# elte-collective-intelligence/student-mechanism-design

Measured on NVIDIA B200. Metric: batched_env_steps_per_sec, higher is better.
Workload: dtype int32/f64

## Files before the change

### include/sy_env.h

```cpp
#ifndef SY_ENV_H
#define SY_ENV_H

#include <stdint.h>

#ifdef __cplusplus
extern "C" {
#endif

#define SY_ABI_VERSION 4
#define SY_NUM_REWARD_WEIGHTS 11
#define SY_MAX_AGENTS 16
#define SY_NUM_STATS 16
#define SY_MAX_COPY_SEGMENTS 8
#define SY_DEFAULT_ACTION (-1)

enum {
  SY_OK = 0,
  SY_ERR_INVALID_ARGUMENT = 1,
  SY_ERR_CUDA = 2,
  SY_ERR_STATE = 3
};

enum { SY_REWARD_FP64 = 0, SY_REWARD_FP32 = 1 };
enum { SY_STATUS_TERMINATED = 1, SY_STATUS_TRUNCATED = 2, SY_STATUS_FROZEN = 4 };
// ... 67 lines not shown
  int32_t* mrx_revealed;
  uint8_t* node_features_u8;
} SyObs;

typedef struct SyOut {
  uint64_t struct_bytes;
  float* reward;
  double* reward64;
  uint8_t* terminated;
  uint8_t* truncated;
  uint8_t* done;
  int8_t* winner;
  int64_t* stats;
  uint8_t* status;
} SyOut;

int sy_abi_version(void);
const char* sy_last_error(void);
int64_t sy_launch_count(void);

int sy_create(const SyConfig* config, SyEnv** out_env);
void sy_destroy(SyEnv* env);
enum { SY_OPT_WRITER_PATH = 0, SY_OPT_STEP_KERNEL = 1, SY_OPT_NF_FILL = 2, SY_OPT_LAGGED_KERNEL = 3, SY_OPT_TAIL_SPLIT = 4,
       SY_OPT_ROLLOUT_KERNEL = 5, SY_OPT_PDL = 6 };
enum { SY_WRITER_BULK = 0, SY_WRITER_LSU = 1 };
enum { SY_STEP_FUSED = 0, SY_STEP_TWO_KERNELS = 1, SY_STEP_AUTO = 2 };
enum { SY_LAGGED_OFF = 0, SY_LAGGED_ON = 1, SY_LAGGED_AUTO = 2 };
int sy_set_option(SyEnv* env, int32_t option, int32_t value);
int sy_set_seed(SyEnv* env, uint64_t seed);

int sy_set_reward_tables(SyEnv* env, const double* exp_neg, int32_t n_exp, const double* coverage,
                         int32_t n_cov, sy_stream_t stream);

int sy_load_graphs(SyEnv* env, int32_t num_graphs, const int32_t* row_ptr, const int32_t* col,
                   const int32_t* w, int32_t nnz_stride, sy_stream_t stream);
int sy_generate_graphs(SyEnv* env, int32_t num_graphs, int32_t num_edges, int32_t max_edges_per_node, int32_t max_weight,
                       uint64_t seed, uint32_t generation, uint32_t graph_offset, int32_t* attempts_host,
                       sy_stream_t stream);
int sy_read_graph_edges(SyEnv* env, int32_t* edge_links, int32_t* weights, int32_t* counts, int32_t max_edges,
                        sy_stream_t stream);
int sy_read_graph_tables(SyEnv* env, int32_t g, uint8_t* weights, uint16_t* apsp, sy_stream_t stream);

int sy_reset(SyEnv* env, const uint8_t* reset_mask, const int32_t* init_pos, const int32_t* init_graph_id,
             int32_t restart, const SyState* state, const SyObs* obs, sy_stream_t stream);

int sy_step(SyEnv* env, const int64_t* actions, const SyState* state, const SyObs* obs, const SyOut* out,
            sy_stream_t stream);

int sy_step_deferred(SyEnv* env, const int64_t* actions, const SyState* state, const SyObs* obs, const SyOut* out,
                     sy_stream_t stream);
int sy_flush_observations(SyEnv* env, const SyState* state, const SyObs* obs, sy_stream_t stream);
int sy_observations_pending(SyEnv* env);

typedef struct SyHostOut {
  uint64_t struct_bytes;
  float* reward;
  uint8_t* terminated;
  uint8_t* truncated;
  uint8_t* done;
  int8_t* winner;
  uint8_t* status;
} SyHostOut;

int sy_step_host(SyEnv* env, const int64_t* actions_host, int64_t* actions_dev, const SyState* state,
                 const SyObs* obs, const SyOut* out, const SyHostOut* host_out, sy_stream_t stream);

int sy_step_i32(SyEnv* env, const int32_t* actions, const SyState* state, const SyObs* obs, const SyOut* out,
                sy_stream_t stream);
int sy_step_i16(SyEnv* env, const int16_t* actions, const SyState* state, const SyObs* obs, const SyOut* out,
                sy_stream_t stream);
int sy_step_host_i16(SyEnv* env, const int16_t* actions_host, int16_t* actions_dev, const SyState* state,
                     const SyObs* obs, const SyOut* out, const SyHostOut* host_out, sy_stream_t stream);
int sy_sample_actions_i16(SyEnv* env, const SyState* state, uint32_t step_counter, int16_t* actions,
                          sy_stream_t stream);
int sy_set_host_overlap(SyEnv* env, int32_t on);
// ... 46 lines not shown
```

### student_mechanism_design_b200/_cabi.py

```python
from __future__ import annotations

import ctypes as C
import os

_HERE = os.path.dirname(os.path.abspath(__file__))
LIB_PATH = os.environ.get("SY_LIB_PATH") or os.path.join(_HERE, "libsy_env.so")

SY_ABI_VERSION = 4
SY_NUM_REWARD_WEIGHTS = 11
SY_MAX_AGENTS = 16
SY_NUM_STATS = 16
SY_MAX_GROUPS = 1024
SY_REWARD_FP64, SY_REWARD_FP32 = 0, 1
STAT_NAMES = [
    "env_steps", "episodes", "mrx_wins", "police_wins", "truncations", "out_of_money",
    "sum_episode_length", "sum_budget_spent", "sum_sq_episode_length", "sum_length_police_wins",
    "sum_length_mrx_wins", "sum_episode_budget_spent", "police_moves",
    "reveals", "sum_belief_ce_q24", "sum_sq_belief_ce_q24",
]
BELIEF_CE_SCALE = float(1 << 24)


class SyConfig(C.Structure):
    _fields_ = [
# ... 45 lines not shown
    "sy_launch_count": (C.c_int64, []),
    "sy_create": (C.c_int, [C.POINTER(SyConfig), C.POINTER(C.c_void_p)]),
    "sy_destroy": (None, [C.c_void_p]),
    "sy_set_option": (C.c_int, [C.c_void_p, C.c_int32, C.c_int32]),
    "sy_set_seed": (C.c_int, [C.c_void_p, C.c_uint64]),
    "sy_set_reward_tables": (C.c_int, [C.c_void_p, C.c_void_p, C.c_int32, C.c_void_p, C.c_int32, C.c_void_p]),
    "sy_load_graphs": (C.c_int, [C.c_void_p, C.c_int32, C.c_void_p, C.c_void_p, C.c_void_p, C.c_int32, C.c_void_p]),
    "sy_read_graph_tables": (C.c_int, [C.c_void_p, C.c_int32, C.c_void_p, C.c_void_p, C.c_void_p]),
    "sy_generate_graphs": (C.c_int, [C.c_void_p, C.c_int32, C.c_int32, C.c_int32, C.c_int32, C.c_uint64, C.c_uint32,
                                     C.c_uint32, C.c_void_p, C.c_void_p]),
    "sy_read_graph_edges": (C.c_int, [C.c_void_p, C.c_void_p, C.c_void_p, C.c_void_p, C.c_int32, C.c_void_p]),
    "sy_reset": (C.c_int, [C.c_void_p, C.c_void_p, C.c_void_p, C.c_void_p, C.c_int32, C.POINTER(SyState),
                           C.POINTER(SyObs), C.c_void_p]),
    "sy_step": (C.c_int, [C.c_void_p, C.c_void_p, C.POINTER(SyState), C.POINTER(SyObs), C.POINTER(SyOut), C.c_void_p]),
    "sy_step_host": (C.c_int, [C.c_void_p, C.c_void_p, C.c_void_p, C.POINTER(SyState), C.POINTER(SyObs), C.POINTER(SyOut),
                               C.POINTER(SyHostOut), C.c_void_p]),
    "sy_step_i16": (C.c_int, [C.c_void_p, C.c_void_p, C.POINTER(SyState), C.POINTER(SyObs), C.POINTER(SyOut), C.c_void_p]),
    "sy_step_host_i16": (C.c_int, [C.c_void_p, C.c_void_p, C.c_void_p, C.POINTER(SyState), C.POINTER(SyObs),
                                   C.POINTER(SyOut), C.POINTER(SyHostOut), C.c_void_p]),
    "sy_sample_actions_i16": (C.c_int, [C.c_void_p, C.POINTER(SyState), C.c_uint32, C.c_void_p, C.c_void_p]),
    "sy_step_deferred": (C.c_int, [C.c_void_p, C.c_void_p, C.POINTER(SyState), C.POINTER(SyObs), C.POINTER(SyOut), C.c_void_p]),
    "sy_flush_observations": (C.c_int, [C.c_void_p, C.POINTER(SyState), C.POINTER(SyObs), C.c_void_p]),
    "sy_observations_pending": (C.c_int, [C.c_void_p]),
    "sy_step_i32": (C.c_int, [C.c_void_p, C.c_void_p, C.POINTER(SyState), C.POINTER(SyObs), C.POINTER(SyOut), C.c_void_p]),
    "sy_step_host_i32": (C.c_int, [C.c_void_p, C.c_void_p, C.c_void_p, C.POINTER(SyState), C.POINTER(SyObs),
                                   C.POINTER(SyOut), C.POINTER(SyHostOut), C.c_void_p]),
    "sy_set_host_overlap": (C.c_int, [C.c_void_p, C.c_int32]),
    "sy_host_rollout_random": (C.c_int, [C.c_void_p, C.c_int32, C.c_uint32, C.c_void_p, C.c_void_p, C.c_int32, C.POINTER(SyState),
                                         C.POINTER(SyObs), C.POINTER(SyOut), C.POINTER(SyHostOut), C.c_void_p]),
    "sy_sample_actions_host": (C.c_int, [C.c_void_p, C.POINTER(SyState), C.c_uint32, C.c_void_p, C.c_void_p, C.c_int32, C.c_void_p]),
    "sy_sample_actions_i32": (C.c_int, [C.c_void_p, C.POINTER(SyState), C.c_uint32, C.c_void_p, C.c_void_p]),
    "sy_sample_actions": (C.c_int, [C.c_void_p, C.POINTER(SyState), C.c_uint32, C.c_void_p, C.c_void_p]),
    "sy_copy_segments": (C.c_int, [C.c_int32, C.c_void_p, C.c_void_p, C.c_void_p, C.c_void_p]),
    "sy_stats": (C.c_int, [C.c_void_p, C.c_void_p, C.c_void_p]),
    "sy_set_groups": (C.c_int, [C.c_void_p, C.c_int32, C.POINTER(SyGroup), C.c_void_p, C.c_void_p]),
    "sy_group_stats": (C.c_int, [C.c_void_p, C.c_int32, C.c_void_p, C.c_void_p]),
    "sy_allreduce_stats": (C.c_int, [C.c_void_p, C.c_void_p, C.c_void_p, C.c_void_p, C.c_void_p]),
    "sy_rollout_random_dev": (C.c_int, [C.c_void_p, C.c_int32, C.c_void_p, C.c_void_p, C.POINTER(SyState), C.POINTER(SyObs),
                                        C.POINTER(SyOut), C.c_void_p]),
    "sy_rollout_random": (C.c_int, [C.c_void_p, C.c_int32, C.c_uint32, C.c_void_p, C.POINTER(SyState), C.POINTER(SyObs),
                                    C.POINTER(SyOut), C.c_void_p]),
    "sy_action_mask_dense": (C.c_int, [C.c_int32, C.c_int32, C.c_void_p, C.c_void_p, C.c_void_p, C.c_double,
                                       C.c_void_p, C.c_void_p, C.c_void_p, C.c_void_p]),
}

_lib = None
# ... 29 lines not shown
```

### student_mechanism_design_b200/csrc/sy_env.cu

```cuda
#include "../../include/sy_env.h"

#include <cuda_runtime.h>
#include <dlfcn.h>

#include <algorithm>
#include <atomic>
#include <cstdarg>
#include <cstdio>
#include <cstdlib>
#include <cmath>
#include <cstring>
#include <mutex>
#include <string>
#include <vector>

namespace {

thread_local std::string g_err;
std::atomic<long long> g_launches{0};

int fail(int code, const char* fmt, ...) {
  char buf[512];
  va_list ap;
  va_start(ap, fmt);
// ... 89 lines not shown
  int bel_share_csr;
  int wr_img_rows;
  int wr_off_pad;
  int wr_bulk, wr_c_mask, wr_c_nf, wr_img_bytes;
  int nf_prefilled;
  int f_off_sbuf, f_sbuf_stride, f_off_zero, f_off_imgs;
  int f_off_nbr4;
  int wr_epc;
  int ob_full, ob_split;
  int dbg_skip;
  unsigned long long* stats_rep;
  uint8_t* bel_flags;
  long long* next_actions;
  unsigned next_counter;
  const unsigned* next_counter_base;
  const uint8_t* reset_mask;
  const int32_t* init_pos;
  const int32_t* init_gid;
  int restart;
  const struct GroupRow* grp;
  const int32_t* grp_id;
  int grp_n, grp_rep;
  unsigned long long* grp_stats;
};

struct GroupRow {
  double w64[SY_NUM_REWARD_WEIGHTS];
  float w32[SY_NUM_REWARD_WEIGHTS];
  int agent_money, reveal;
  unsigned long long reveal_skip_thresh;
};


#ifdef SY_FUSED_CLOCKS
__device__ unsigned long long g_fused_clk[16];
#define FCLK_ADD(slot, v) do { if (lane == 0) atomicAdd(&g_fused_clk[slot], (unsigned long long)(v)); } while (0)
#define FCLK_NOW() clock64()
#else
#define FCLK_ADD(slot, v) do { } while (0)
#define FCLK_NOW() 0ll
#pragma nv_diag_suppress 177
#endif

__device__ __forceinline__ uint4 philox4x32(uint4 c, uint2 k) {
#pragma unroll
  for (int r = 0; r < 10; ++r) {
// ... 53 lines not shown

__device__ __forceinline__ int edge_weight(const Tables& tb, int N, int g, int u, int v) {
  return __ldg(tb.W + ((size_t)g * N + u) * tb.Ns + v);
}
__device__ __forceinline__ int move_count(const Tables& tb, int N, int g, int u, int money, int toll) {
  int c = money - toll;
  if (c <= 0) return 0;
  c = min(c, tb.wcap);
  return __ldg(tb.cnt + ((size_t)g * N + u) * (tb.wcap + 1) + c);
}
__device__ __forceinline__ double exp_neg(const Tables& tb, int d) {
  return (d < tb.n_exp) ? __ldg(tb.exp_neg + d) : 0.0;
}

__device__ __forceinline__ void store_obs16(uint4* ptr, uint4 v) {
#if SY_STORE_HINT == 0
  __stcs(ptr, v);
#elif SY_STORE_HINT == 1
  *ptr = v;
#elif SY_STORE_HINT == 2
  __stcg(ptr, v);
#else
  __stwt(ptr, v);
#endif
}
__device__ __forceinline__ void cp_async4(void* smem, const void* gmem) {
  const unsigned sa = (unsigned)__cvta_generic_to_shared(smem);
  asm volatile("cp.async.ca.shared.global [%0], [%1], 4;\n" ::"r"(sa), "l"(gmem));
}
__device__ __forceinline__ void cp_async16(void* smem, const void* gmem) {
  const unsigned sa = (unsigned)__cvta_generic_to_shared(smem);
  asm volatile("cp.async.cg.shared.global [%0], [%1], 16;\n" ::"r"(sa), "l"(gmem));
}
__device__ __forceinline__ void cp_async_wait_all() { asm volatile("cp.async.wait_all;\n" ::: "memory"); }
__device__ __forceinline__ void pdl_wait() { asm volatile("griddepcontrol.wait;\n" ::: "memory"); }
__device__ __forceinline__ void pdl_launch_dependents() { asm volatile("griddepcontrol.launch_dependents;\n" ::: "memory"); }
__device__ __forceinline__ void named_barrier(int id, int nthreads) {
  asm volatile("bar.sync %0, %1;\n" ::"r"(id), "r"(nthreads) : "memory");
}

__device__ __forceinline__ void fence_proxy_async_smem() { asm volatile("fence.proxy.async.shared::cta;\n" ::: "memory"); }
__device__ __forceinline__ void bulk_store(void* gdst, const void* ssrc, unsigned bytes) {
  const unsigned sa = (unsigned)__cvta_generic_to_shared(ssrc);
#if SY_BULK_HINT == 1
  unsigned long long pol;
  asm volatile("createpolicy.fractional.L2::evict_first.b64 %0, 1.0;\n" : "=l"(pol));
// ... 747 lines not shown
#else
  if (lane < A) {
    const int f0 = fpos[lane] - head;
    if (fpos[lane] >= 0 && f0 >= 0 && f0 < (nvec << 2)) {
      const int myc = f0 >> 2;
      uint4 v = z;
      for (int a = 0; a < A; ++a) {
        const int f = fpos[a] - head;
        if (fpos[a] >= 0 && (f >> 2) == myc) {
          const unsigned one = 0x3f800000u;
          const int sub = f & 3;
          v.x = sub == 0 ? one : v.x;
          v.y = sub == 1 ? one : v.y;
          v.z = sub == 2 ? one : v.z;
          v.w = sub == 3 ? one : v.w;
        }
      }
      store_obs16(body + myc, v);
    }
  }
#endif
}

template <int WRW, bool PREFILLED = false, int LAGT = 0, int CSRT = 0>
__device__ __forceinline__ void writer_role(const Params& p, unsigned char* dyn, int tile0, int nEnv, int w, int lane,
                                            int* lag_staged = nullptr) {
  const Tables& tb = p.tb;
  const int N = p.N, A = p.A;
  int* s_pos = reinterpret_cast<int*>(dyn + p.wr_off);
  int* s_money = s_pos + TILE * A;
  int* s_rev = s_money + TILE * A;
  int* s_gid = s_rev + TILE;
  int* s_fpos = s_gid + TILE;
  uint8_t* s_img = reinterpret_cast<uint8_t*>(s_fpos + WRW * SY_MAX_AGENTS) + (size_t)w * p.wr_img_stride;
  int* s_rp = reinterpret_cast<int*>(dyn + p.wr_off_csr);
  uint16_t* s_col = reinterpret_cast<uint16_t*>(s_rp + N + 1);
  uint8_t* s_wgt = reinterpret_cast<uint8_t*>(s_col + tb.nnz_stride);
  const int tw = w * 32 + lane;
  const int gl = (lane < nEnv) ? p.st.graph_id[tile0 + lane] : -1;
  const int g0 = __shfl_sync(FULL, gl, 0);
  const bool staged = p.wr_stage_csr && __all_sync(FULL, gl == g0 || gl < 0);
  for (int i = tw; i < nEnv * A; i += WRW * 32) {
    s_pos[i] = p.st.pos[(size_t)tile0 * A + i];
    s_money[i] = p.st.money[(size_t)tile0 * A + i];
  }
  if (tw < nEnv) {
    s_rev[tw] = p.ob.mrx_revealed[tile0 + tw];
    s_gid[tw] = gl;
  }
  if (staged) {
    const int32_t* grp = tb.row_ptr + (size_t)g0 * (N + 1);
    const int nnz = __ldg(grp + N);
    for (int i = tw; i <= N; i += WRW * 32) s_rp[i] = __ldg(grp + i);
    for (int k = tw; k < nnz; k += WRW * 32) {
      s_col[k] = __ldg(tb.col + (size_t)g0 * tb.nnz_stride + k);
      s_wgt[k] = __ldg(tb.wgt + (size_t)g0 * tb.nnz_stride + k);
    }
    if (p.bel_share_csr) {
      float* s_inv = reinterpret_cast<float*>(dyn + p.wr_off_csr + (((N + 1) * 4 + tb.nnz_stride * 3 + 3) & ~3));
      uint16_t* s_perm = reinterpret_cast<uint16_t*>(s_inv + N);
      for (int i = tw; i < N; i += WRW * 32) {
// ... 6 lines not shown
      const int2* gpk = tb.nbr_pack + (size_t)g0 * tb.pack_stride;
      const int npk = __ldg(gpp + N);
      for (int i = tw; i <= N; i += WRW * 32) s_pptr[i] = (uint16_t)__ldg(gpp + i);
      for (int k = tw; k < npk; k += WRW * 32) {
        const int2 en = __ldg(gpk + k);
        s_pcol[k] = en.y ? (uint16_t)((unsigned)en.x / (BSTRIDE * 4u)) : (uint16_t)N;
      }
    }
  }
  for (int i = lane * 16; i < p.wr_img_stride; i += 32 * 16) *reinterpret_cast<uint4*>(s_img + i) = make_uint4(0, 0, 0, 0);
  if constexpr (CSRT > 0) {
    if (tw == 0) *lag_staged = staged ? 1 : 0;
  }
  named_barrier(2, WRW * 32);
  if (p.bel_share_csr) asm volatile("bar.arrive 3, %0;\n" ::"r"(THREADS) : "memory");
  if constexpr (CSRT > 0) asm volatile("bar.arrive %0, %1;\n" ::"n"(LAG_CSR_BAR), "n"(CSRT) : "memory");
  if constexpr (LAGT > 0) asm volatile("bar.arrive %0, %1;\n" ::"n"(LAG_BAR), "n"(LAGT) : "memory");
  int* fpos = s_fpos + w * SY_MAX_AGENTS;
  const int R = p.wr_img_rows;
  const int lpa = R == 1 ? 32 : 32 / A;
  for (int e = w; e < nEnv; e += WRW) {
    const int b = tile0 + e;
    float* nf = p.ob.node_features + (size_t)b * N * A;
    if (lane < A) fpos[lane] = (lane > 0 || s_rev[e] >= 0) ? s_pos[e * A + lane] * A + lane : -1;
    for (int a0 = 0; a0 < A; a0 += R) {
      uint8_t* mask = p.ob.action_mask + ((size_t)b * A + a0) * N;
      const int phase = (int)(reinterpret_cast<uintptr_t>(mask) & 15u);
      uint8_t* img = s_img + phase;
      const int ag = a0 + lane / lpa, sub = lane % lpa;
      if (ag < A && lane / lpa < R && !(p.dbg_skip & 2)) {
        const int u = s_pos[e * A + ag], m = s_money[e * A + ag], g = s_gid[e];
        uint8_t* row = img + (ag - a0) * N;
        if (staged) {
          const int r0 = s_rp[u], r1 = s_rp[u + 1];
          for (int k = r0 + sub; k < r1; k += lpa)
            if ((int)s_wgt[k] + p.toll <= m) row[s_col[k]] = 1;
        } else {
          const int32_t* rp = tb.row_ptr + (size_t)g * (N + 1) + u;
          const int r0 = __ldg(rp), r1 = __ldg(rp + 1);
          const uint16_t* cl = tb.col + (size_t)g * tb.nnz_stride;
          const uint8_t* wg = tb.wgt + (size_t)g * tb.nnz_stride;
          for (int k = r0 + sub; k < r1; k += lpa)
            if ((int)__ldg(wg + k) + p.toll <= m) row[__ldg(cl + k)] = 1;
        }
      }
      __syncwarp();
      warp_copy_bytes(mask, img, min(R, A - a0) * N, lane);
      if (a0 + R < A) {
        __syncwarp();
        for (int i = lane * 16; i < p.wr_img_stride; i += 32 * 16) *reinterpret_cast<uint4*>(s_img + i) = make_uint4(0, 0, 0, 0);
        __syncwarp();
      }
    }
    __syncwarp();
    if (p.ob.node_features_u8 && R != A) {
      uint8_t* nf8 = p.ob.node_features_u8 + (size_t)b * N * A;
      warp_zero_bytes(nf8, N * A, lane);
      __syncwarp();
      if (lane < A && fpos[lane] >= 0) nf8[fpos[lane]] = 1;
    } else if (p.ob.node_features_u8) {
      __syncwarp();
      for (int i = lane * 16; i < p.wr_img_stride; i += 32 * 16) *reinterpret_cast<uint4*>(s_img + i) = make_uint4(0, 0, 0, 0);
      __syncwarp();
      uint8_t* nf8 = p.ob.node_features_u8 + (size_t)b * N * A;
      uint8_t* img8 = s_img + (int)(reinterpret_cast<uintptr_t>(nf8) & 15u);
      if (lane < A && fpos[lane] >= 0) img8[fpos[lane]] = 1;
      __syncwarp();
      warp_copy_bytes(nf8, img8, N * A, lane);
    } else {
      if constexpr (PREFILLED) warp_write_node_feature_ones(nf, N * A, fpos, A, lane);
      else warp_write_node_features(nf, N * A, fpos, A, lane);
    }
    __syncwarp();
    for (int i = lane * 16; i < p.wr_img_stride; i += 32 * 16) *reinterpret_cast<uint4*>(s_img + i) = make_uint4(0, 0, 0, 0);
    __syncwarp();
  }
}

struct BulkCtx {
  const int* s_pos;
  const int* s_money;
  const int* s_rev;
  const int* s_gid;
  const int* rp;
  const uint16_t* col;
  const uint8_t* wgt;
};

template <bool STAGED>
__device__ __forceinline__ void bulk_mask_ones(const Params& p, const BulkCtx& c, uint8_t* img, int lo, int len, int lane, uint8_t v) {
  const int N = p.N, A = p.A, S = A * N;
  const int e_lo = lo / S, e_hi = (lo + len - 1) / S;
  const int npairs = (e_hi - e_lo + 1) * A;
  for (int q = lane; q < npairs; q += 32) {
    const int de = (q * p.inv_A) >> 16, a = q - de * A, e = e_lo + de;
// ... 206 lines not shown
      const int32_t* gpp = tb.pack_ptr + (size_t)g0 * (N + 1);
      const int2* gpk = tb.nbr_pack + (size_t)g0 * tb.pack_stride;
      const int npk = __ldg(gpp + N);
      for (int i = tw; i <= N; i += NTHREADS) s_pptr[i] = (uint16_t)__ldg(gpp + i);
      for (int k = tw; k < npk; k += NTHREADS) {
        const int2 en = __ldg(gpk + k);
        s_pcol[k] = en.y ? (uint16_t)((unsigned)en.x / (BSTRIDE * 4u)) : (uint16_t)N;
      }
    }
  }
  return staged;
}

template <int WRW>
__device__ __forceinline__ void writer_role_bulk(const Params& p, unsigned char* dyn, int tile0, int nEnv, int w, int lane) {
  constexpr int NW = WRW < BULK_WARPS ? WRW : BULK_WARPS;
  const int N = p.N, A = p.A;
  int* s_pos = reinterpret_cast<int*>(dyn + p.wr_off);
  int* s_money = s_pos + TILE * A;
  int* s_rev = s_money + TILE * A;
  int* s_gid = s_rev + TILE;
  uint8_t* zero_page = reinterpret_cast<uint8_t*>(s_gid + TILE);
  uint8_t* imgs = zero_page + p.wr_img_bytes;
  for (int i = (w * 32 + lane) * 16; i < (1 + 2 * NW) * p.wr_img_bytes; i += WRW * 32 * 16) *reinterpret_cast<uint4*>(zero_page + i) = make_uint4(0, 0, 0, 0);
  fence_proxy_async_smem();
  const bool staged = stage_tile_inputs<WRW * 32>(p, dyn, tile0, nEnv, w * 32 + lane, lane, s_pos, s_money, s_rev, s_gid);
  named_barrier(2, WRW * 32);
  if (p.bel_share_csr) asm volatile("bar.arrive 3, %0;\n" ::"r"(THREADS) : "memory");
  if (w >= NW) return;
  int* s_rp = reinterpret_cast<int*>(dyn + p.wr_off_csr);
  uint16_t* s_col = reinterpret_cast<uint16_t*>(s_rp + N + 1);
  const BulkCtx c{s_pos, s_money, s_rev, s_gid, s_rp, s_col, reinterpret_cast<uint8_t*>(s_col + p.tb.nnz_stride)};
  const ImageStreams st = image_streams(p, tile0, nEnv);
  uint8_t* gnf32 = p.ob.node_features_u8 ? nullptr : reinterpret_cast<uint8_t*>(p.ob.node_features) + (size_t)tile0 * N * A * 4;
  writer_stream_warp<BULK_DEPTH>(p, c, st, staged, imgs + (size_t)w * 2 * p.wr_img_bytes, zero_page, gnf32, w, NW, lane, false);
}

struct CeAcc {
  int n = 0;
  long long sum_q = 0, sq_q = 0;
};
constexpr float CE_CLIP = 1e-8f;
constexpr float CE_Q = 16777216.0f;

__device__ __forceinline__ float ce_clip(float v) { return fminf(fmaxf(v, CE_CLIP), 1.0f); }

// ... 506 lines not shown
  if (deg > 1 && (int)(nb.y >> 16) <= lim) row[nb.y & 0xffffu] = v;
  if (deg > 2 && (int)(nb.z >> 16) <= lim) row[nb.z & 0xffffu] = v;
  if (deg > 3 && (int)(nb.w >> 16) <= lim) row[nb.w & 0xffffu] = v;
  if (deg > 4) {
    const int r0 = s_rp[pv.u];
    for (int k = r0 + 4; k < r0 + deg; ++k)
      if ((int)s_wgt[k] <= lim) row[s_col[k]] = v;
  }
}
__device__ __forceinline__ void fast_nf32_ones(const Params& p, const PairView& pv, const int* s_rev, uint8_t* gnf, int lane) {
  const int A = p.A;
  if (pv.valid && !(pv.a == 0 && s_rev[pv.e] < 0))
    __stcs(reinterpret_cast<float*>(gnf + (size_t)pv.e * p.N * A * 4) + pv.u * A + pv.a, 1.0f);
}

template <int BW>
__device__ __forceinline__ void fused_writer_role(const Params& p, unsigned char* dyn, const unsigned* tiles_done, int w, int lane) {
  constexpr int D = BULK_DEPTH;
  const Tables& tb = p.tb;
  const int N = p.N, A = p.A;
  const int ntiles = (p.B + TILE - 1) / TILE;
  const int nk = ((int)blockIdx.x < ntiles) ? (ntiles - 1 - (int)blockIdx.x) / (int)gridDim.x + 1 : 0;
  if (nk == 0) return;
  const int Cm = p.wr_c_mask;
  const bool nf8 = p.ob.node_features_u8 != nullptr;
  const size_t Sm = (size_t)A * N;
  uint8_t* zero_page = dyn + p.f_off_zero;
  uint8_t* my_img = dyn + p.f_off_imgs + (size_t)w * 2 * p.wr_img_bytes;
  int* s_rp = reinterpret_cast<int*>(dyn + p.wr_off_csr);
  uint16_t* s_col = reinterpret_cast<uint16_t*>(s_rp + N + 1);
  uint8_t* s_wgt = reinterpret_cast<uint8_t*>(s_col + tb.nnz_stride);
  uint4* s_nbr4 = reinterpret_cast<uint4*>(dyn + p.f_off_nbr4);
  const int tw = w * 32 + lane;
  for (int i = tw * 16; i < (1 + 2 * FUSED_WR) * p.wr_img_bytes; i += FUSED_WR * 32 * 16) *reinterpret_cast<uint4*>(zero_page + i) = make_uint4(0, 0, 0, 0);
  fence_proxy_async_smem();
  named_barrier(2, FUSED_WR * 32);
  auto tile_of = [&](int k) { return (int)blockIdx.x + k * (int)gridDim.x; };
  auto envs_of = [&](int k) { return min(TILE, p.B - tile_of(k) * TILE); };
  auto gnf_of = [&](int k) { return reinterpret_cast<uint8_t*>(p.ob.node_features) + (size_t)tile_of(k) * TILE * Sm * 4; };
  auto sbuf = [&](int k) { return reinterpret_cast<int*>(dyn + p.f_off_sbuf + (size_t)(k & 1) * p.f_sbuf_stride); };
  auto ctx_of = [&](int k) {
    int* b = sbuf(k);
    return BulkCtx{b, b + TILE * A, b + 2 * TILE * A, b + 2 * TILE * A + TILE, s_rp, s_col, s_wgt};
  };
  auto fill_piece = [&](uint8_t* g, int Tf32, int cm) {
    const int lo = 4 * cm * Cm, hi = min(Tf32, lo + 4 * Cm);
// ... 604 lines not shown
  int A = 0;
  bool graphs_loaded = false;
  bool tables_set = false;
  Tables tb{};
  void* d_W = nullptr;
  void* d_D = nullptr;
  void* d_row_ptr = nullptr;
  void* d_col = nullptr;
  void* d_wgt = nullptr;
  void* d_cnt = nullptr;
  void* d_inv_deg = nullptr;
  void* d_pack = nullptr;
  void* d_pack_ptr = nullptr;
  void* d_deg_perm = nullptr;
  void* d_edges = nullptr;
  void* d_edge_w = nullptr;
  void* d_edge_count = nullptr;
  void* d_gen_status = nullptr;
  void* d_gen_want = nullptr;
  int gen_max_edges = 0;
  int alloc_G = 0, alloc_nnz = 0, alloc_wcap = 0, alloc_pack = 0;
  void* d_bel_flags = nullptr;
  void* d_stats_rep = nullptr;
  cudaStream_t aux_stream = nullptr;
  int host_overlap = 0;
  bool aux_after_logic = false;
  cudaEvent_t ev_main = nullptr;
  cudaEvent_t ev_fork = nullptr, ev_join = nullptr;
  cudaEvent_t ev_logic = nullptr, ev_copied = nullptr;
  void* d_exp = nullptr;
  void* d_cov = nullptr;
  size_t bel_smem = 0;
  int bel_fast = 0, bel_off_out = 0, bel_off_part = 0, bel_off_pack = 0, bel_off_ptr = 0;
  int wr_off = 0, wr_off_csr = 0, wr_img_stride = 0, wr_stage_csr = 0, bel_share_csr = 0, wr_img_rows = 0, wr_off_pad = 0;
  int wr_c_mask = 0, wr_c_nf32 = 0, wr_c_nf8 = 0, wr_img_bytes = 0;
  bool fused_ok = false;
  int f_bw = 0, f_off_sbuf = 0, f_sbuf_stride = 0, f_off_zero = 0, f_off_imgs = 0, f_off_csr = 0, f_c_mask = 0, f_img_bytes = 0;
  int f_stage_csr = 0, f_grid = 0, f_epc = 0, f_off_nbr4 = 0;
  size_t f_smem = 0;
  int opt_fused = SY_STEP_AUTO;
  int opt_fill = 0;
  cudaStream_t split_stream = nullptr;
  cudaEvent_t ev_split_start = nullptr, ev_split_logic = nullptr, ev_split_belief = nullptr;
  int fill_grid = 0;
  int opt_writer = SY_WRITER_LSU;
  int bel_warps = BEL_WARPS, wr_warps = WR_WARPS;
// ... 297 lines not shown
  p.bel_flags = (uint8_t*)env->d_bel_flags;
  p.stats_rep = (unsigned long long*)env->d_stats_rep;
  p.bel_fast = env->bel_fast;
  p.bel_off_out = env->bel_off_out;
  p.bel_off_part = env->bel_off_part;
  p.bel_off_pack = env->bel_off_pack;
  p.bel_off_ptr = env->bel_off_ptr;
  p.wr_off = env->wr_off;
  p.wr_off_csr = env->wr_off_csr;
  p.wr_img_stride = env->wr_img_stride;
  p.wr_stage_csr = env->wr_stage_csr;
  p.wr_img_rows = env->wr_img_rows;
  p.wr_off_pad = env->wr_off_pad;
  p.bel_share_csr = (p.dbg_skip & 5) ? 0 : env->bel_share_csr;
  p.st = *st;
  if (ob) p.ob = *ob;
  if (out) p.out = *out;
  if (ob) {
    const uintptr_t bits = reinterpret_cast<uintptr_t>(ob->action_mask) | reinterpret_cast<uintptr_t>(ob->node_features_u8 ? (void*)ob->node_features_u8 : (void*)ob->node_features);
    p.wr_bulk = (env->opt_writer == SY_WRITER_BULK && (bits & 15u) == 0) ? 1 : 0;
    p.wr_c_mask = env->wr_c_mask;
    p.wr_c_nf = ob->node_features_u8 ? env->wr_c_nf8 : env->wr_c_nf32;
    p.wr_img_bytes = env->wr_img_bytes;
  }
  if (env->grp_n) {
    p.grp = (const GroupRow*)env->d_grp;
    p.grp_id = (const int32_t*)env->d_grp_id;
    p.grp_n = env->grp_n;
    p.grp_rep = env->grp_rep;
    p.grp_stats = (unsigned long long*)env->d_grp_stats;
  }
  return SY_OK;
}



int check_obs(const SyObs* ob) {
  if (ob && ob->struct_bytes != sizeof(SyObs)) return fail(SY_ERR_INVALID_ARGUMENT, "SyObs size mismatch: got %llu, library expects %zu (ABI %d)", (unsigned long long)ob->struct_bytes, sizeof(SyObs), SY_ABI_VERSION);
  if (!ob || !ob->action_mask || (!ob->node_features && !ob->node_features_u8) || !ob->agent_budget || !ob->mrx_revealed)
    return fail(SY_ERR_INVALID_ARGUMENT, "SyObs has NULL members");
  return SY_OK;
}

}

extern "C" {

// ... 27 lines not shown
  if (!c || !out_env) return fail(SY_ERR_INVALID_ARGUMENT, "NULL config / out_env");
  if (c->struct_bytes != (int32_t)sizeof(SyConfig))
    return fail(SY_ERR_INVALID_ARGUMENT, "SyConfig size mismatch: got %d, library expects %zu", c->struct_bytes, sizeof(SyConfig));
  if (c->num_envs <= 0) return fail(SY_ERR_INVALID_ARGUMENT, "num_envs must be positive");
  if ((long long)c->num_envs * (c->num_police + 1) >= (1LL << 31)) return fail(SY_ERR_INVALID_ARGUMENT, "num_envs x agents must stay below 2^31 per handle");
  if (c->num_police < 1 || c->num_police + 1 > SY_MAX_AGENTS)
    return fail(SY_ERR_INVALID_ARGUMENT, "num_police must be in [1, %d]", SY_MAX_AGENTS - 1);
  if (c->num_nodes < c->num_police + 1 || c->num_nodes > 65534)
    return fail(SY_ERR_INVALID_ARGUMENT, "num_nodes must be in [num_police + 1, 65534]");
  if (c->agent_money < 0 || c->mrx_money < 0 || c->toll < 0 || c->reveal_interval < 0 || c->max_timestep < 0)
    return fail(SY_ERR_INVALID_ARGUMENT, "negative money / toll / reveal_interval / max_timestep");
  if (!(c->reveal_skip_prob >= 0.0f && c->reveal_skip_prob <= 1.0f)) return fail(SY_ERR_INVALID_ARGUMENT, "reveal_skip_prob must be in [0, 1]");
  if (c->reward_mode != SY_REWARD_FP64 && c->reward_mode != SY_REWARD_FP32)
    return fail(SY_ERR_INVALID_ARGUMENT, "unknown reward_mode %d", c->reward_mode);
  int ndev = 0;
  CUDA_TRY(cudaGetDeviceCount(&ndev));
  if (c->device < 0 || c->device >= ndev) return fail(SY_ERR_INVALID_ARGUMENT, "device %d out of range (%d visible)", c->device, ndev);
  CUDA_TRY(cudaSetDevice(c->device));
  SyEnv* e = new SyEnv();
  e->cfg = *c;
  e->A = c->num_police + 1;
  if (cudaMalloc(&e->d_bel_flags, (size_t)c->num_envs) != cudaSuccess ||
      cudaMalloc(&e->d_stats_rep, (size_t)STAT_REPLICAS * SY_NUM_STATS * sizeof(unsigned long long)) != cudaSuccess ||
      cudaMemset(e->d_stats_rep, 0, (size_t)STAT_REPLICAS * SY_NUM_STATS * sizeof(unsigned long long)) != cudaSuccess) {
    sy_destroy(e);
    return fail(SY_ERR_CUDA, "cudaMalloc of the per-env flag / statistics buffers failed");
  }
  if (cudaStreamCreateWithFlags(&e->aux_stream, cudaStreamNonBlocking) != cudaSuccess ||
      cudaEventCreateWithFlags(&e->ev_logic, cudaEventDisableTiming) != cudaSuccess ||
      cudaEventCreateWithFlags(&e->ev_copied, cudaEventDisableTiming) != cudaSuccess) {
    sy_destroy(e);
    return fail(SY_ERR_CUDA, "stream / event creation failed");
  }
  *out_env = e;
  return SY_OK;
}

void sy_destroy(SyEnv* e) {
  if (!e) return;
  cudaSetDevice(e->cfg.device);
  free_graph_tables(e);
  if (e->d_exp) cudaFree(e->d_exp);
  if (e->d_cov) cudaFree(e->d_cov);
  if (e->d_bel_flags) cudaFree(e->d_bel_flags);
  if (e->d_stats_rep) cudaFree(e->d_stats_rep);
  for (void* ptr : {e->d_grp, e->d_grp_id, e->d_grp_id_new, e->d_grp_bad, e->d_grp_stats})
    if (ptr) cudaFree(ptr);
  if (e->aux_stream) cudaStreamDestroy(e->aux_stream);
  if (e->split_stream) cudaStreamDestroy(e->split_stream);
  for (cudaEvent_t ev : {e->ev_split_start, e->ev_split_logic, e->ev_split_belief})
    if (ev) cudaEventDestroy(ev);
  if (e->ev_main) cudaEventDestroy(e->ev_main);
  if (e->ev_fork) cudaEventDestroy(e->ev_fork);
  if (e->ev_join) cudaEventDestroy(e->ev_join);
  if (e->ev_logic) cudaEventDestroy(e->ev_logic);
  if (e->ev_copied) cudaEventDestroy(e->ev_copied);
  delete e;
}

int sy_set_option(SyEnv* e, int32_t option, int32_t value) {
  if (!e) return fail(SY_ERR_INVALID_ARGUMENT, "NULL env");
  switch (option) {
    case SY_OPT_STEP_KERNEL:
      if (value != SY_STEP_FUSED && value != SY_STEP_TWO_KERNELS && value != SY_STEP_AUTO)
        return fail(SY_ERR_INVALID_ARGUMENT, "SY_OPT_STEP_KERNEL: 0 (fused), 1 (two kernels) or 2 (auto)");
      e->opt_fused = value;
      return SY_OK;
    case SY_OPT_NF_FILL:
      if (value != 0 && value != 1) return fail(SY_ERR_INVALID_ARGUMENT, "SY_OPT_NF_FILL: 0 or 1");
      e->opt_fill = value;
      return SY_OK;
    case SY_OPT_WRITER_PATH:
      if (value != SY_WRITER_BULK && value != SY_WRITER_LSU) return fail(SY_ERR_INVALID_ARGUMENT, "SY_OPT_WRITER_PATH: 0 (bulk) or 1 (LSU)");
      e->opt_writer = value;
      return SY_OK;
    case SY_OPT_PDL:
      if (value != 0 && value != 1) return fail(SY_ERR_INVALID_ARGUMENT, "SY_OPT_PDL: 0 or 1");
      e->opt_pdl = value;
      return SY_OK;
    case SY_OPT_ROLLOUT_KERNEL:
      if (value != 0 && value != 1) return fail(SY_ERR_INVALID_ARGUMENT, "SY_OPT_ROLLOUT_KERNEL: 0 or 1");
      e->opt_rollout_kernel = value;
      return SY_OK;
    case SY_OPT_TAIL_SPLIT:
      if (value != 0 && value != 1) return fail(SY_ERR_INVALID_ARGUMENT, "SY_OPT_TAIL_SPLIT: 0 or 1");
      e->opt_tail_split = value;
      return SY_OK;
    case SY_OPT_LAGGED_KERNEL:
      if (value != SY_LAGGED_OFF && value != SY_LAGGED_ON && value != SY_LAGGED_AUTO)
        return fail(SY_ERR_INVALID_ARGUMENT, "SY_OPT_LAGGED_KERNEL: 0 (off), 1 (on) or 2 (auto)");
      e->opt_lagged = value;
      return SY_OK;
    default:
      return fail(SY_ERR_INVALID_ARGUMENT, "unknown option %d", option);
  }
}

int sy_set_seed(SyEnv* e, uint64_t seed) {
  if (!e) return fail(SY_ERR_INVALID_ARGUMENT, "NULL env");
  e->cfg.seed = seed;
  return SY_OK;
}

int sy_set_reward_tables(SyEnv* e, const double* exp_neg_h, int32_t n_exp, const double* cov_h, int32_t n_cov, sy_stream_t stream) {
  if (!e || !exp_neg_h || !cov_h || n_exp < 1 || n_cov < 2) return fail(SY_ERR_INVALID_ARGUMENT, "bad reward tables");
  if (n_exp > DIST_INF) n_exp = DIST_INF;
  CUDA_TRY(cudaSetDevice(e->cfg.device));
  cudaStream_t s = (cudaStream_t)stream;
  if (e->d_exp) cudaFree(e->d_exp);
  if (e->d_cov) cudaFree(e->d_cov);
  e->d_exp = e->d_cov = nullptr;
  CUDA_TRY(cudaMalloc(&e->d_exp, (size_t)n_exp * sizeof(double)));
  CUDA_TRY(cudaMalloc(&e->d_cov, (size_t)n_cov * sizeof(double)));
  CUDA_TRY(cudaMemcpyAsync(e->d_exp, exp_neg_h, (size_t)n_exp * sizeof(double), cudaMemcpyHostToDevice, s));
// ... 542 lines not shown

int sy_step_deferred(SyEnv* e, const int64_t* actions, const SyState* st, const SyObs* ob, const SyOut* out, sy_stream_t stream) {
  return step_impl(e, actions, nullptr, st, ob, out, stream, nullptr, nullptr, nullptr, 0, nullptr, nullptr, true);
}

int sy_flush_observations(SyEnv* e, const SyState* st, const SyObs* ob, sy_stream_t stream) {
  if (!e) return fail(SY_ERR_INVALID_ARGUMENT, "NULL env");
  if (!e->obs_pending) return SY_OK;
  Params p;
  int rc = fill_params(e, st, ob, nullptr, p);
  if (rc) return rc;
  if ((rc = check_obs(ob))) return rc;
  p.out.stats = e->pending_stats;
  CUDA_TRY(cudaSetDevice(e->cfg.device));
  launch_observe(e, p, (unsigned)((p.B + TILE - 1) / TILE), (cudaStream_t)stream);
  g_launches++;
  CUDA_TRY(cudaGetLastError());
  e->obs_pending = false;
  return SY_OK;
}

int sy_observations_pending(SyEnv* e) { return e && e->obs_pending ? 1 : 0; }

int sy_step_i32(SyEnv* e, const int32_t* actions, const SyState* st, const SyObs* ob, const SyOut* out, sy_stream_t stream) {
  return step_impl(e, nullptr, actions, st, ob, out, stream);
}

int sy_step_host(SyEnv* e, const int64_t* actions_host, int64_t* actions_dev, const SyState* st, const SyObs* ob,
                 const SyOut* out, const SyHostOut* ho, sy_stream_t stream) {
  if (!e || !actions_host || !actions_dev || !ho) return fail(SY_ERR_INVALID_ARGUMENT, "NULL env / actions / host_out");
  if (ho->struct_bytes != sizeof(SyHostOut)) return fail(SY_ERR_INVALID_ARGUMENT, "SyHostOut size mismatch: got %llu, library expects %zu (ABI %d)", (unsigned long long)ho->struct_bytes, sizeof(SyHostOut), SY_ABI_VERSION);
  CUDA_TRY(cudaSetDevice(e->cfg.device));
  cudaStream_t s = (cudaStream_t)stream;
  const size_t n = (size_t)e->cfg.num_envs * e->A;
  CUDA_TRY(cudaMemcpyAsync(actions_dev, actions_host, n * sizeof(int64_t), cudaMemcpyHostToDevice, s));
  const int rc = step_impl(e, actions_dev, nullptr, st, ob, out, stream, e->ev_logic);
  if (rc) return rc;
  return copy_results_and_sync(e, out, ho, s);
}

int sy_step_host_i32(SyEnv* e, const int32_t* actions_host, int32_t* actions_dev, const SyState* st, const SyObs* ob,
                     const SyOut* out, const SyHostOut* ho, sy_stream_t stream) {
  if (!e || !actions_host || !actions_dev || !ho) return fail(SY_ERR_INVALID_ARGUMENT, "NULL env / actions / host_out");
  if (ho->struct_bytes != sizeof(SyHostOut)) return fail(SY_ERR_INVALID_ARGUMENT, "SyHostOut size mismatch: got %llu, library expects %zu (ABI %d)", (unsigned long long)ho->struct_bytes, sizeof(SyHostOut), SY_ABI_VERSION);
  CUDA_TRY(cudaSetDevice(e->cfg.device));
  cudaStream_t s = (cudaStream_t)stream;
// ... 333 lines not shown
```

### student_mechanism_design_b200/env.py

```python
from __future__ import annotations

import ctypes as C
from typing import Dict, List, Optional, Sequence

import numpy as np
import torch

from . import _cabi
from .graphs import GraphSpec, generate_graph_pool, pack_csr

REWARD_WEIGHT_NAMES = [
    "Police_distance", "Police_group", "Police_position", "Police_time", "Mrx_closest", "Mrx_average",
    "Mrx_position", "Mrx_time", "Police_coverage", "Police_proximity", "Police_overlap_penalty",
]
DEFAULT_REWARD_WEIGHTS = {
    "Police_distance": 0.1, "Police_group": 0.1, "Police_position": 0.1, "Police_time": 0.0,
    "Mrx_closest": 0.3, "Mrx_average": 0.2, "Mrx_position": 0.1, "Mrx_time": 0.0,
    "Police_coverage": 0.05, "Police_proximity": 0.05, "Police_overlap_penalty": 0.0,
}
GRAPH_BLOCK = 32
MAX_MONEY_LIMIT = 1000
N_EXP_TABLE = 1100


# ... 107 lines not shown
            self.num_graphs = len(self.graphs)
        self.graph_edges = graph_edges
        N, A, B = self.graph_nodes, self.num_agents, self.num_envs

        cfg = _cabi.SyConfig()
        cfg.struct_bytes = C.sizeof(_cabi.SyConfig)
        cfg.device, cfg.num_envs, cfg.num_nodes, cfg.num_police = dev_index, B, N, self.number_of_agents
        cfg.agent_money, cfg.mrx_money, cfg.max_timestep = self.agent_money, MAX_MONEY_LIMIT, int(max_timestep)
        cfg.reveal_interval, cfg.toll = int(reveal_interval or 0), int(tolls)
        cfg.belief = 2 if (belief and belief_ce) else int(bool(belief))
        cfg.reward_mode = _cabi.SY_REWARD_FP32 if reward_mode == "fp32" else _cabi.SY_REWARD_FP64
        cfg.auto_reset, cfg.resample_graph = int(bool(auto_reset)), int(bool(resample_graph))
        cfg.env_offset, cfg.seed = int(env_offset), int(seed) & 0xFFFFFFFFFFFFFFFF
        cfg.reveal_skip_prob = float(reveal_skip_prob)
        for i, v in enumerate(wvals):
            cfg.reward_weights[i] = v
        self.config = cfg
        self.reveal_interval, self.tolls, self.belief_on = cfg.reveal_interval, cfg.toll, bool(cfg.belief)
        self.auto_reset, self.seed, self.env_offset = bool(auto_reset), int(seed), int(env_offset)

        self._handle = C.c_void_p()
        with torch.cuda.device(self.device):
            _cabi.check(self._lib.sy_create(C.byref(cfg), C.byref(self._handle)))
            stream = self._stream()
            exp_neg, coverage = reward_tables if reward_tables is not None else numpy_reward_tables(max_timestep)
            exp_neg = np.ascontiguousarray(exp_neg, dtype=np.float64)
            coverage = np.ascontiguousarray(coverage, dtype=np.float64)
            _cabi.check(self._lib.sy_set_reward_tables(self._handle, exp_neg.ctypes.data, len(exp_neg),
                                                       coverage.ctypes.data, len(coverage), stream))
            if self._device_pool:
                self._generate_on_device(0)
            else:
                row_ptr, col, wgt, stride = pack_csr(self.graphs)
                self._csr = (row_ptr, col, wgt)
                _cabi.check(self._lib.sy_load_graphs(self._handle, self.num_graphs, row_ptr.ctypes.data, col.ctypes.data,
                                                     wgt.ctypes.data, stride, stream))

            dev = self.device
            self._guards = []
            guard = (int(guard_bytes) + 255) & ~255

            def z(*shape, dtype):
                if not guard:
                    return torch.zeros(*shape, dtype=dtype, device=dev)
                n = 1
                for d in shape:
# ... 62 lines not shown
        return torch.cuda.current_stream(self.device).cuda_stream

    def close(self):
        if getattr(self, "_handle", None) is not None and self._handle:
            self._lib.sy_destroy(self._handle)
            self._handle = None

    def __del__(self):
        try:
            self.close()
        except Exception:
            pass

    def _dev(self, x, dtype, shape):
        t = torch.as_tensor(x)
        t = t.to(device=self.device, dtype=dtype).contiguous()
        if tuple(t.shape) != tuple(shape):
            raise ValueError(f"expected shape {tuple(shape)}, got {tuple(t.shape)}")
        return t

    OPTIONS = {"writer_path": (0, {"bulk": 0, "lsu": 1}), "step_kernel": (1, {"fused": 0, "two_kernels": 1, "auto": 2}),
               "nf_fill": (2, {"off": 0, "on": 1}), "lagged_kernel": (3, {"off": 0, "on": 1, "auto": 2}),
               "tail_split": (4, {"off": 0, "on": 1}), "rollout_kernel": (5, {"off": 0, "on": 1}),
               "pdl": (6, {"off": 0, "on": 1})}

    def set_option(self, name: str, value):
        opt, values = self.OPTIONS[name]
        _cabi.check(self._lib.sy_set_option(self._handle, opt, values[value] if isinstance(value, str) else int(value)))
        self.options = dict(getattr(self, "options", {}), **{name: value})

    def set_belief_hint(self, hint: Optional[torch.Tensor]):
        if hint is not None:
            if not self.belief_on:
                raise _cabi.SyError("belief hints need belief=True")
            hint = hint.to(device=self.device).contiguous()
            if hint.dtype == torch.bool:
                hint = hint.view(torch.uint8)
            if hint.dtype != torch.uint8 or tuple(hint.shape) != (self.num_envs, self.graph_nodes):
                raise ValueError(f"hint must be uint8/bool [{self.num_envs}, {self.graph_nodes}]")
        self._belief_hint = hint
        self._state.belief_hint = _ptr(hint)

    def set_seed(self, seed: int):
        self.seed = int(seed)
        self.config.seed = self.seed & 0xFFFFFFFFFFFFFFFF
        _cabi.check(self._lib.sy_set_seed(self._handle, self.config.seed))

# ... 396 lines not shown
            self._fold_stats()
            self.stats_vec.zero_()
            if self.group_stats_vec is not None:
                self.group_stats_vec.zero_()

    def state_dict(self) -> Dict[str, torch.Tensor]:
        keys = ["pos", "money", "timestep", "graph_id", "episode", "done", "visits", "belief_map", "action_mask",
                "node_features", "agent_budget", "mrx_revealed", "stats_vec"]
        self._fold_stats()
        sd = {k: getattr(self, k).clone() for k in keys if getattr(self, k) is not None}
        if self._group_id is not None:
            sd["group_id"] = self._group_id.clone()
            if self.group_stats_vec is not None:
                sd["group_stats_vec"] = self.group_stats_vec.clone()
        return sd

    def load_state_dict(self, sd: Dict[str, torch.Tensor]):
        if ("group_id" in sd) != (self._group_id is not None) or (
                "group_id" in sd and not torch.equal(sd["group_id"].to(self._group_id.device), self._group_id)):
            raise ValueError("the state dict's mechanism groups differ from this env's: set_mechanisms() first")
        for k, v in sd.items():
            if k != "group_id":
                getattr(self, k).copy_(v)
        self._is_reset = True


class _RolloutGraph:

    def __init__(self, graph, env):
        self.graph, self._env, self._generation = graph, env, env._groups_generation

    def replay(self):
        if self._env._groups_generation != self._generation:
            raise _cabi.SyError("the mechanism groups changed since this rollout graph was captured: capture it again")
        self.graph.replay()

    def __getattr__(self, name):
        return getattr(self.graph, name)


class _LazyGather:

    def __init__(self, table: torch.Tensor, gid: torch.Tensor):
        self.table, self.gid = table, gid
        self.shape = (gid.shape[0],) + tuple(table.shape[1:])

    def __getitem__(self, idx):
# ... 33 lines not shown
```

Before: 505.2 million.

## Write node-feature observations as deltas from a per-env shadow of last positions

Adds a per-env shadow of the agent nodes last written into node_features plus a tag recording which buffer and dtype were written. When the tag matches, the writer clears only the old agent entries and sets the new ones with aligned 32-byte stores, skipping the full zero-and-rewrite of the N*A feature block. It is enabled by default from Python. The cost is extra shadow and tag loads and stores per env, plus the risk of stale features if the buffer is changed outside the env, which load_state_dict covers by invalidating.

Result: faster. 518.6 million (median of 6 runs) (+2.7%).

```diff
diff --git a/include/sy_env.h b/include/sy_env.h
--- a/include/sy_env.h
+++ b/include/sy_env.h
@@ -113,7 +113,7 @@
 int sy_create(const SyConfig* config, SyEnv** out_env);
 void sy_destroy(SyEnv* env);
 enum { SY_OPT_WRITER_PATH = 0, SY_OPT_STEP_KERNEL = 1, SY_OPT_NF_FILL = 2, SY_OPT_LAGGED_KERNEL = 3, SY_OPT_TAIL_SPLIT = 4,
-       SY_OPT_ROLLOUT_KERNEL = 5, SY_OPT_PDL = 6 };
+       SY_OPT_ROLLOUT_KERNEL = 5, SY_OPT_PDL = 6, SY_OPT_NF_DELTA = 7 };
 enum { SY_WRITER_BULK = 0, SY_WRITER_LSU = 1 };
 enum { SY_STEP_FUSED = 0, SY_STEP_TWO_KERNELS = 1, SY_STEP_AUTO = 2 };
 enum { SY_LAGGED_OFF = 0, SY_LAGGED_ON = 1, SY_LAGGED_AUTO = 2 };
@@ -142,6 +142,7 @@
                      sy_stream_t stream);
 int sy_flush_observations(SyEnv* env, const SyState* state, const SyObs* obs, sy_stream_t stream);
 int sy_observations_pending(SyEnv* env);
+int sy_invalidate_observations(SyEnv* env, sy_stream_t stream);
 
 typedef struct SyHostOut {
   uint64_t struct_bytes;
diff --git a/student_mechanism_design_b200/_cabi.py b/student_mechanism_design_b200/_cabi.py
--- a/student_mechanism_design_b200/_cabi.py
+++ b/student_mechanism_design_b200/_cabi.py
@@ -91,6 +91,7 @@
     "sy_step_deferred": (C.c_int, [C.c_void_p, C.c_void_p, C.POINTER(SyState), C.POINTER(SyObs), C.POINTER(SyOut), C.c_void_p]),
     "sy_flush_observations": (C.c_int, [C.c_void_p, C.POINTER(SyState), C.POINTER(SyObs), C.c_void_p]),
     "sy_observations_pending": (C.c_int, [C.c_void_p]),
+    "sy_invalidate_observations": (C.c_int, [C.c_void_p, C.c_void_p]),
     "sy_step_i32": (C.c_int, [C.c_void_p, C.c_void_p, C.POINTER(SyState), C.POINTER(SyObs), C.POINTER(SyOut), C.c_void_p]),
     "sy_step_host_i32": (C.c_int, [C.c_void_p, C.c_void_p, C.c_void_p, C.POINTER(SyState), C.POINTER(SyObs),
                                    C.POINTER(SyOut), C.POINTER(SyHostOut), C.c_void_p]),
diff --git a/student_mechanism_design_b200/csrc/sy_env.cu b/student_mechanism_design_b200/csrc/sy_env.cu
--- a/student_mechanism_design_b200/csrc/sy_env.cu
+++ b/student_mechanism_design_b200/csrc/sy_env.cu
@@ -135,6 +135,9 @@
   const int32_t* grp_id;
   int grp_n, grp_rep;
   unsigned long long* grp_stats;
+  uint16_t* nf_shadow;
+  unsigned long long* nf_tag;
+  unsigned long long nf_tag_want;
 };
 
 struct GroupRow {
@@ -234,6 +237,15 @@
   __stcg(ptr, v);
 #else
   __stwt(ptr, v);
+#endif
+}
+__device__ __forceinline__ void store_obs32(void* ptr, const unsigned (&v)[8]) {
+#if SY_STORE_HINT == 0
+  asm volatile("st.global.cs.v8.b32 [%0], {%1, %2, %3, %4, %5, %6, %7, %8};\n" ::"l"(ptr), "r"(v[0]), "r"(v[1]), "r"(v[2]),
+               "r"(v[3]), "r"(v[4]), "r"(v[5]), "r"(v[6]), "r"(v[7]) : "memory");
+#else
+  asm volatile("st.global.v8.b32 [%0], {%1, %2, %3, %4, %5, %6, %7, %8};\n" ::"l"(ptr), "r"(v[0]), "r"(v[1]), "r"(v[2]),
+               "r"(v[3]), "r"(v[4]), "r"(v[5]), "r"(v[6]), "r"(v[7]) : "memory");
 #endif
 }
 __device__ __forceinline__ void cp_async4(void* smem, const void* gmem) {
@@ -1027,6 +1039,44 @@
 #endif
 }
 
+template <int ES>
+__device__ __forceinline__ void warp_delta_node_features(uint8_t* base, int n, const int* fpos, int old_node, int A, int lane) {
+  const int a = lane < A ? lane : lane - A;
+  const int oldn = __shfl_sync(FULL, old_node, a & 31);
+  const int fnew = lane < 2 * A ? fpos[a] : -1;
+  const int fold = oldn == 0xFFFF ? -1 : oldn * A + a;
+  const int f = (lane < 2 * A && fold != fnew) ? (lane < A ? fold : fnew) : -1;
+  const int ph = (int)(reinterpret_cast<uintptr_t>(base) & 31u);
+  const int sb = (((ph + f * ES) >> 5) << 5) - ph;
+  unsigned v[8];
+#pragma unroll
+  for (int k = 0; k < 8; ++k) v[k] = 0u;
+#pragma unroll
+  for (int q = 0; q < SY_MAX_AGENTS; ++q) {
+    const int fq = q < A ? fpos[q] : -1;
+    const int o = fq * ES - sb;
+    if (fq >= 0 && o >= 0 && o < 32) {
+      const unsigned bits = ES == 4 ? 0x3f800000u : 1u << ((o & 3) * 8);
+#pragma unroll
+      for (int k = 0; k < 8; ++k) v[k] |= (o >> 2) == k ? bits : 0u;
+    }
+  }
+  if (f < 0) return;
+  const int nb = n * ES;
+  if (sb >= 0 && sb + 32 <= nb) {
+    store_obs32(base + sb, v);
+  } else {
+#pragma unroll
+    for (int k = 0; k < 32 / ES; ++k) {
+      const int o = sb + k * ES;
+      if (o >= 0 && o < nb) {
+        if constexpr (ES == 4) *reinterpret_cast<unsigned*>(base + o) = v[k];
+        else base[o] = (uint8_t)(v[k >> 2] >> ((k & 3) * 8));
+      }
+    }
+  }
+}
+
 template <int WRW, bool PREFILLED = false, int LAGT = 0, int CSRT = 0>
 __device__ __forceinline__ void writer_role(const Params& p, unsigned char* dyn, int tile0, int nEnv, int w, int lane,
                                             int* lag_staged = nullptr) {
@@ -1042,6 +1092,13 @@
   uint16_t* s_col = reinterpret_cast<uint16_t*>(s_rp + N + 1);
   uint8_t* s_wgt = reinterpret_cast<uint8_t*>(s_col + tb.nnz_stride);
   const int tw = w * 32 + lane;
+  const unsigned long long want = p.nf_tag_want;
+  unsigned long long tag_next = 0ull;
+  int old_next = 0xFFFF;
+  if (want && w < nEnv) {
+    tag_next = p.nf_tag[tile0 + w];
+    if (lane < A) old_next = p.nf_shadow[(size_t)(tile0 + w) * A + lane];
+  }
   const int gl = (lane < nEnv) ? p.st.graph_id[tile0 + lane] : -1;
   const int g0 = __shfl_sync(FULL, gl, 0);
   const bool staged = p.wr_stage_csr && __all_sync(FULL, gl == g0 || gl < 0);
@@ -1094,7 +1151,14 @@
   for (int e = w; e < nEnv; e += WRW) {
     const int b = tile0 + e;
     float* nf = p.ob.node_features + (size_t)b * N * A;
-    if (lane < A) fpos[lane] = (lane > 0 || s_rev[e] >= 0) ? s_pos[e * A + lane] * A + lane : -1;
+    const int new_node = (lane < A && (lane > 0 || s_rev[e] >= 0)) ? s_pos[e * A + lane] : 0xFFFF;
+    if (lane < A) fpos[lane] = new_node == 0xFFFF ? -1 : new_node * A + lane;
+    const bool delta = !PREFILLED && want && tag_next == want;
+    const int old_node = old_next;
+    if (want && e + WRW < nEnv) {
+      tag_next = p.nf_tag[b + WRW];
+      if (lane < A) old_next = p.nf_shadow[(size_t)(b + WRW) * A + lane];
+    }
     for (int a0 = 0; a0 < A; a0 += R) {
       uint8_t* mask = p.ob.action_mask + ((size_t)b * A + a0) * N;
       const int phase = (int)(reinterpret_cast<uintptr_t>(mask) & 15u);
@@ -1125,7 +1189,10 @@
       }
     }
     __syncwarp();
-    if (p.ob.node_features_u8 && R != A) {
+    if (delta) {
+      if (p.ob.node_features_u8) warp_delta_node_features<1>(p.ob.node_features_u8 + (size_t)b * N * A, N * A, fpos, old_node, A, lane);
+      else warp_delta_node_features<4>(reinterpret_cast<uint8_t*>(nf), N * A, fpos, old_node, A, lane);
+    } else if (p.ob.node_features_u8 && R != A) {
       uint8_t* nf8 = p.ob.node_features_u8 + (size_t)b * N * A;
       warp_zero_bytes(nf8, N * A, lane);
       __syncwarp();
@@ -1143,6 +1210,8 @@
       if constexpr (PREFILLED) warp_write_node_feature_ones(nf, N * A, fpos, A, lane);
       else warp_write_node_features(nf, N * A, fpos, A, lane);
     }
+    if (want && lane < A && (!delta || old_node != new_node)) p.nf_shadow[(size_t)b * A + lane] = (uint16_t)new_node;
+    if (!delta && lane == 0) p.nf_tag[b] = want;
     __syncwarp();
     for (int i = lane * 16; i < p.wr_img_stride; i += 32 * 16) *reinterpret_cast<uint4*>(s_img + i) = make_uint4(0, 0, 0, 0);
     __syncwarp();
@@ -1395,6 +1464,7 @@
   int* s_gid = s_rev + TILE;
   uint8_t* zero_page = reinterpret_cast<uint8_t*>(s_gid + TILE);
   uint8_t* imgs = zero_page + p.wr_img_bytes;
+  if (w == 0 && lane < nEnv) p.nf_tag[tile0 + lane] = 0;
   for (int i = (w * 32 + lane) * 16; i < (1 + 2 * NW) * p.wr_img_bytes; i += WRW * 32 * 16) *reinterpret_cast<uint4*>(zero_page + i) = make_uint4(0, 0, 0, 0);
   fence_proxy_async_smem();
   const bool staged = stage_tile_inputs<WRW * 32>(p, dyn, tile0, nEnv, w * 32 + lane, lane, s_pos, s_money, s_rev, s_gid);
@@ -1947,6 +2017,9 @@
   const int ntiles = (p.B + TILE - 1) / TILE;
   const int nk = ((int)blockIdx.x < ntiles) ? (ntiles - 1 - (int)blockIdx.x) / (int)gridDim.x + 1 : 0;
   if (nk == 0) return;
+  if (w == 0)
+    for (int k = 0; k < nk; ++k)
+      if (lane < min(TILE, p.B - ((int)blockIdx.x + k * (int)gridDim.x) * TILE)) p.nf_tag[((int)blockIdx.x + k * (int)gridDim.x) * TILE + lane] = 0;
   const int Cm = p.wr_c_mask;
   const bool nf8 = p.ob.node_features_u8 != nullptr;
   const size_t Sm = (size_t)A * N;
@@ -2597,6 +2670,9 @@
   int alloc_G = 0, alloc_nnz = 0, alloc_wcap = 0, alloc_pack = 0;
   void* d_bel_flags = nullptr;
   void* d_stats_rep = nullptr;
+  void* d_nf_shadow = nullptr;
+  void* d_nf_tag = nullptr;
+  int opt_nf_delta = 0;
   cudaStream_t aux_stream = nullptr;
   int host_overlap = 0;
   bool aux_after_logic = false;
@@ -2940,7 +3016,12 @@
     p.wr_c_mask = env->wr_c_mask;
     p.wr_c_nf = ob->node_features_u8 ? env->wr_c_nf8 : env->wr_c_nf32;
     p.wr_img_bytes = env->wr_img_bytes;
-  }
+    const void* nfp = ob->node_features_u8 ? (const void*)ob->node_features_u8 : (const void*)ob->node_features;
+    const uintptr_t nfa = reinterpret_cast<uintptr_t>(nfp);
+    p.nf_tag_want = (env->opt_nf_delta && nfa && (nfa & 15u) == 0) ? (unsigned long long)nfa | (ob->node_features_u8 ? 2ull : 1ull) : 0ull;
+  }
+  p.nf_shadow = (uint16_t*)env->d_nf_shadow;
+  p.nf_tag = (unsigned long long*)env->d_nf_tag;
   if (env->grp_n) {
     p.grp = (const GroupRow*)env->d_grp;
     p.grp_id = (const int32_t*)env->d_grp_id;
@@ -3014,9 +3095,12 @@
   e->A = c->num_police + 1;
   if (cudaMalloc(&e->d_bel_flags, (size_t)c->num_envs) != cudaSuccess ||
       cudaMalloc(&e->d_stats_rep, (size_t)STAT_REPLICAS * SY_NUM_STATS * sizeof(unsigned long long)) != cudaSuccess ||
-      cudaMemset(e->d_stats_rep, 0, (size_t)STAT_REPLICAS * SY_NUM_STATS * sizeof(unsigned long long)) != cudaSuccess) {
+      cudaMemset(e->d_stats_rep, 0, (size_t)STAT_REPLICAS * SY_NUM_STATS * sizeof(unsigned long long)) != cudaSuccess ||
+      cudaMalloc(&e->d_nf_shadow, (size_t)c->num_envs * e->A * sizeof(uint16_t)) != cudaSuccess ||
+      cudaMalloc(&e->d_nf_tag, (size_t)c->num_envs * sizeof(unsigned long long)) != cudaSuccess ||
+      cudaMemset(e->d_nf_tag, 0, (size_t)c->num_envs * sizeof(unsigned long long)) != cudaSuccess) {
     sy_destroy(e);
-    return fail(SY_ERR_CUDA, "cudaMalloc of the per-env flag / statistics buffers failed");
+    return fail(SY_ERR_CUDA, "cudaMalloc of the per-env flag / statistics / node_features record buffers failed");
   }
   if (cudaStreamCreateWithFlags(&e->aux_stream, cudaStreamNonBlocking) != cudaSuccess ||
       cudaEventCreateWithFlags(&e->ev_logic, cudaEventDisableTiming) != cudaSuccess ||
@@ -3036,6 +3120,8 @@
   if (e->d_cov) cudaFree(e->d_cov);
   if (e->d_bel_flags) cudaFree(e->d_bel_flags);
   if (e->d_stats_rep) cudaFree(e->d_stats_rep);
+  if (e->d_nf_shadow) cudaFree(e->d_nf_shadow);
+  if (e->d_nf_tag) cudaFree(e->d_nf_tag);
   for (void* ptr : {e->d_grp, e->d_grp_id, e->d_grp_id_new, e->d_grp_bad, e->d_grp_stats})
     if (ptr) cudaFree(ptr);
   if (e->aux_stream) cudaStreamDestroy(e->aux_stream);
@@ -3082,6 +3168,10 @@
       if (value != SY_LAGGED_OFF && value != SY_LAGGED_ON && value != SY_LAGGED_AUTO)
         return fail(SY_ERR_INVALID_ARGUMENT, "SY_OPT_LAGGED_KERNEL: 0 (off), 1 (on) or 2 (auto)");
       e->opt_lagged = value;
+      return SY_OK;
+    case SY_OPT_NF_DELTA:
+      if (value != 0 && value != 1) return fail(SY_ERR_INVALID_ARGUMENT, "SY_OPT_NF_DELTA: 0 or 1");
+      e->opt_nf_delta = value;
       return SY_OK;
     default:
       return fail(SY_ERR_INVALID_ARGUMENT, "unknown option %d", option);
@@ -3670,6 +3760,13 @@
 
 int sy_observations_pending(SyEnv* e) { return e && e->obs_pending ? 1 : 0; }
 
+int sy_invalidate_observations(SyEnv* e, sy_stream_t stream) {
+  if (!e) return fail(SY_ERR_INVALID_ARGUMENT, "NULL env");
+  CUDA_TRY(cudaSetDevice(e->cfg.device));
+  CUDA_TRY(cudaMemsetAsync(e->d_nf_tag, 0, (size_t)e->cfg.num_envs * sizeof(unsigned long long), (cudaStream_t)stream));
+  return SY_OK;
+}
+
 int sy_step_i32(SyEnv* e, const int32_t* actions, const SyState* st, const SyObs* ob, const SyOut* out, sy_stream_t stream) {
   return step_impl(e, nullptr, actions, st, ob, out, stream);
 }
diff --git a/student_mechanism_design_b200/env.py b/student_mechanism_design_b200/env.py
--- a/student_mechanism_design_b200/env.py
+++ b/student_mechanism_design_b200/env.py
@@ -153,6 +153,7 @@
         self._handle = C.c_void_p()
         with torch.cuda.device(self.device):
             _cabi.check(self._lib.sy_create(C.byref(cfg), C.byref(self._handle)))
+            _cabi.check(self._lib.sy_set_option(self._handle, self.OPTIONS["nf_delta"][0], 1))
             stream = self._stream()
             exp_neg, coverage = reward_tables if reward_tables is not None else numpy_reward_tables(max_timestep)
             exp_neg = np.ascontiguousarray(exp_neg, dtype=np.float64)
@@ -261,7 +262,7 @@
     OPTIONS = {"writer_path": (0, {"bulk": 0, "lsu": 1}), "step_kernel": (1, {"fused": 0, "two_kernels": 1, "auto": 2}),
                "nf_fill": (2, {"off": 0, "on": 1}), "lagged_kernel": (3, {"off": 0, "on": 1, "auto": 2}),
                "tail_split": (4, {"off": 0, "on": 1}), "rollout_kernel": (5, {"off": 0, "on": 1}),
-               "pdl": (6, {"off": 0, "on": 1})}
+               "pdl": (6, {"off": 0, "on": 1}), "nf_delta": (7, {"off": 0, "on": 1})}
 
     def set_option(self, name: str, value):
         opt, values = self.OPTIONS[name]
@@ -704,7 +705,12 @@
         for k, v in sd.items():
             if k != "group_id":
                 getattr(self, k).copy_(v)
+        self.invalidate_observations()
         self._is_reset = True
+
+    def invalidate_observations(self):
+        with torch.cuda.device(self.device):
+            _cabi.check(self._lib.sy_invalidate_observations(self._handle, self._stream()))
 
 
 class _RolloutGraph:
```
